# kmaninis/OSVOS-PyTorch

Measured on AMD Instinct MI355X. Metric: frames/sec (fwd+bwd) OSVOS-VGG16 854x480 per GPU; mask IoU vs ref, higher is better.
Workload: dtype f32 (3x bf16-split operands on MFMA, f32 accumulate); 1 GPU; 854x480 batch=1 online fine-tune loop (train_online.py), fused-head loss, nAveGrad=5, SGD 8-group, fp32x3, frame resident in HBM; global_batch=1, parallelism=dp1, grad_allreduce=none, rccl_ranks_seen=1

## Files before the change

### osvos-pytorch_amd/csrc/conv3x3_f32x3.hip

```cpp
#include "common.h"
#include "kernels.h"
#include "epi.h"
#include "maskbits.h"
#include "h2split.h"

namespace {

typedef __bf16 bf16x8_t __attribute__((ext_vector_type(8)));
typedef __bf16 bf16x2_t __attribute__((ext_vector_type(2)));
typedef unsigned int u32x4 __attribute__((ext_vector_type(4)));

struct ConvArgsX {
  const float* x;
  const float* wpk;
  const uint4* wpk3;
  const float* bias;
  const float* mask;
  float* y;
  int N, H, W, Cin, Cout, CoutP, y_cs;
  int tiles_x, tiles_y, nct;
  int relu, map, nsp;
  int ksplit;
  float* part;
  ConvEpi epi;
  int sk_order;
  unsigned* sk_tickets;
  float* sk_part;
};

constexpr int cdivx(int a, int b) { return (a + b - 1) / b; }
constexpr int pitch_x(int rbw, int hw) {
  return rbw == 32 ? hw : (rbw == 16 ? cdivx(hw, 16) * 16 : cdivx(hw - 8, 16) * 16 + 8);
}

template <int RBW_, int TBX_, int TBY_, int NB_, int WGM_, int WGN_, int OCC_, int ILV_ = 0>
struct CfgX {
  static constexpr int RBW = RBW_, TBX = TBX_, TBY = TBY_, NB = NB_, WGM = WGM_, WGN = WGN_, OCC = OCC_;
  static constexpr int ILV = ILV_;
  static constexpr int RBH = 32 / RBW;
  static constexpr int TW = TBX * RBW, TH = TBY * RBH;
  static constexpr int HWD = TW + 2, HHT = TH + 2;
  static constexpr int PITCH = pitch_x(RBW, HWD);
  static constexpr int PLANE = HHT * PITCH;
  static constexpr int BN = NB * 32;
  static constexpr int A_U4 = 6 * PLANE;
  static constexpr int B_ITEMS = 18 * BN;
  static constexpr int B_U4 = 3 * B_ITEMS;
  static constexpr int BUF_U4 = A_U4 + B_U4;
  static constexpr int A_ITEMS = HHT * HWD * 2;
  static constexpr int NT = 64 * WGM * WGN;
  static constexpr int NA = cdivx(A_ITEMS, NT);
  static constexpr int NBL = cdivx(B_ITEMS, NT);
  static constexpr int MB = TBX * TBY;
  static constexpr int WM = MB / WGM, WN = NB / WGN;
  static constexpr size_t LDS_BYTES = (size_t)(BUF_U4 + 2) * 16;
  static constexpr int A_U4_2 = 4 * PLANE, B_U4_2 = 2 * B_ITEMS;
  static constexpr size_t LDS_BYTES_2 = (size_t)(A_U4_2 + B_U4_2 + 2 + 4) * 16;
  static constexpr int SK_SLOT_F4 = NT * WM * WN * 4;
  static constexpr int ROW_U4 = 18 * BN;
  static constexpr size_t LDS_BYTES_PIPE = (size_t)(2 * A_U4 + 2 * ROW_U4 + 2) * 16;
  static_assert(WGM * WGN == 4 || WGM * WGN == 8, "4 or 8 waves per workgroup");
  static_assert(MB % WGM == 0 && NB % WGN == 0, "wave grid must divide the tile");
  static_assert(LDS_BYTES <= 160 * 1024, "tile does not fit the 160 KB LDS of a gfx950 CU");
};

__device__ inline unsigned cvt2(float a, float b) {
  bf16x2_t h;
  h[0] = (__bf16)a;
  h[1] = (__bf16)b;
  return __builtin_bit_cast(unsigned, h);
}
__device__ inline void split2(float a, float b, unsigned& p0, unsigned& p1, unsigned& p2) {
  p0 = cvt2(a, b);
  float ra = a - __uint_as_float(p0 << 16), rb = b - __uint_as_float(p0 & 0xffff0000u);
  p1 = cvt2(ra, rb);
  ra -= __uint_as_float(p1 << 16);
  rb -= __uint_as_float(p1 & 0xffff0000u);
  p2 = cvt2(ra, rb);
}
__device__ inline void split8(const u32x4& lo, const u32x4& hi, uint4& p0, uint4& p1, uint4& p2) {
  const f32x4 a = __builtin_bit_cast(f32x4, lo), b = __builtin_bit_cast(f32x4, hi);
  split2(a[0], a[1], p0.x, p1.x, p2.x);
  split2(a[2], a[3], p0.y, p1.y, p2.y);
  split2(b[0], b[1], p0.z, p1.z, p2.z);
  split2(b[2], b[3], p0.w, p1.w, p2.w);
}

__device__ inline void split8_hm(const u32x4& lo, const u32x4& hi, uint4& p0, uint4& p1) {
  const f32x4 a = __builtin_bit_cast(f32x4, lo), b = __builtin_bit_cast(f32x4, hi);
  auto two = [](float x, float y, unsigned& q0, unsigned& q1) {
    q0 = cvt2(x, y);
    q1 = cvt2(x - __uint_as_float(q0 << 16), y - __uint_as_float(q0 & 0xffff0000u));
  };
  two(a[0], a[1], p0.x, p1.x);
  two(a[2], a[3], p0.y, p1.y);
  two(b[0], b[1], p0.z, p1.z);
  two(b[2], b[3], p0.w, p1.w);
}

template <class C, int PS, int SK, int NP = 3, int HP = 0, int PIPE = 0>
__global__ __launch_bounds__(C::NT, C::OCC) void conv3x3_f32x3_kernel(ConvArgsX a) {
  static_assert(NP == 2 || NP == 3, "two or three bf16 pieces per operand");
  static_assert(HP == 0 || (NP == 2 && PS == 1 && SK == 0), "h2: two pieces, pre-split pack, plain grid");
  static_assert(PIPE == 0 || (PS == 1 && NP == 3 && HP == 0 && C::ILV != 0 && C::NT == 512), "pipelined loop: pre-split three-piece eight-wave tiles");
  extern __shared__ __attribute__((aligned(16))) char smem[];
  uint4* As = reinterpret_cast<uint4*>(smem);
  uint4* Bs = As + (NP == 3 ? C::A_U4 : C::A_U4_2);
  const int tid = threadIdx.x, lane = tid & 63, wave = tid >> 6;
  const int li = lane & 31, lh = lane >> 5;
  const int wm = wave / C::WGN, wn = wave % C::WGN;
  const int nch_all = a.Cin >> 4;

  unsigned u = 0, u_end = 0, vme = 0, sk_U = 0, my_first_tile = 0;
  if constexpr (SK != 0) {
    const unsigned G = gridDim.x;
    vme = (G & 7u) == 0 ? (blockIdx.x & 7u) * (G >> 3) + (blockIdx.x >> 3) : blockIdx.x;
    sk_U = (unsigned)(a.nct * a.nsp) * (unsigned)nch_all;
    u = (unsigned)(((unsigned long long)vme * sk_U) / G);
    u_end = (unsigned)(((unsigned long long)(vme + 1) * sk_U) / G);
    my_first_tile = u / (unsigned)nch_all;
  }
 for (;;) {
  int sp, ct;
  int kc_begin, kc_end;
  unsigned tile_id = 0;
  if constexpr (SK != 0) {
    if (u >= u_end) break;
    tile_id = u / (unsigned)nch_all;
    kc_begin = (int)(u - tile_id * (unsigned)nch_all);
    kc_end = min(nch_all, kc_begin + (int)(u_end - u));
    if (a.sk_order == 0) { sp = (int)(tile_id / (unsigned)a.nct); ct = (int)(tile_id % (unsigned)a.nct); }
    else { ct = (int)(tile_id / (unsigned)a.nsp); sp = (int)(tile_id % (unsigned)a.nsp); }
  } else {
    if (a.map == 0) {
      sp = blockIdx.x / a.nct;
      ct = blockIdx.x % a.nct;
    } else {
      const int j = blockIdx.x >> 3;
      ct = j % a.nct;
      sp = (j / a.nct) * 8 + (blockIdx.x & 7);
      if (sp >= a.nsp) return;
    }
    kc_begin = (int)((long)nch_all * blockIdx.y / a.ksplit);
    kc_end = (int)((long)nch_all * (blockIdx.y + 1) / a.ksplit);
  }
  const int tx = sp % a.tiles_x;
  sp /= a.tiles_x;
  const int ty = sp % a.tiles_y;
  const int n = sp / a.tiles_y;
  const int x0 = tx * C::TW, y0 = ty * C::TH, co0 = ct * C::BN;
  const int CQ = a.Cin >> 2;
  const float* ximg = a.x + (size_t)n * a.H * a.W * a.Cin;

  constexpr unsigned OOB = 0x80000000u;
  const __amdgpu_buffer_rsrc_t xrs = __builtin_amdgcn_make_buffer_rsrc(const_cast<float*>(ximg), 0, (int)((size_t)a.H * a.W * a.Cin * 4), 0x00020000);
  const __amdgpu_buffer_rsrc_t wrs = __builtin_amdgcn_make_buffer_rsrc(const_cast<float*>(a.wpk), 0, (int)((size_t)9 * CQ * a.CoutP * 16), 0x00020000);
  unsigned a_off[C::NA];
  int a_dst[C::NA];
#pragma unroll
  for (int i = 0; i < C::NA; ++i) {
    const int e = tid + i * C::NT;
    const int g = e & 1, pix = e >> 1;
    const int hy = pix / C::HWD, hx = pix % C::HWD;
    const int gy = y0 + hy - 1, gx = x0 + hx - 1;
    const bool slot = e < C::A_ITEMS;
    a_dst[i] = slot ? g * C::PLANE + hy * C::PITCH + hx : -1;
    a_off[i] = (slot && gy >= 0 && gy < a.H && gx >= 0 && gx < a.W) ? (unsigned)(((gy * a.W + gx) * a.Cin + 8 * g) * 4) : OOB;
  }
  constexpr int NBI = PS ? cdivx(NP * C::B_ITEMS, C::NT) : C::NBL;
  constexpr int TPI = C::NT / (2 * C::BN);
  static_assert(!PS || C::NT % (2 * C::BN) == 0, "pre-split staging: the thread block must cover whole (piece, tap) rows");
  unsigned b_off[PS ? 1 : C::NBL];
  unsigned b_step = 0;
  int b_row0 = 0;
  if (PS) {
    const int CG = a.Cin >> 3;
    b_row0 = tid / (2 * C::BN);
    const int rem = tid % (2 * C::BN), g = rem / C::BN, nn = rem % C::BN;
    b_off[0] = (co0 + nn < a.CoutP) ? (unsigned)(((b_row0 * CG + g) * a.CoutP + co0 + nn) * 16) : OOB;
    b_step = (unsigned)(TPI * CG * a.CoutP * 16);
  } else {
#pragma unroll
    for (int i = 0; i < C::NBL; ++i) {
      const int e = tid + i * C::NT;
      const int tap = e / (2 * C::BN), rem = e % (2 * C::BN);
      const int g = rem / C::BN, nn = rem % C::BN;
      b_off[i] = (e < C::B_ITEMS && co0 + nn < a.CoutP) ? (unsigned)(((tap * CQ + 2 * g) * a.CoutP + co0 + nn) * 16) : OOB;
    }
  }
  const unsigned b_q1 = (unsigned)a.CoutP * 16u;
  const __amdgpu_buffer_rsrc_t w3rs = __builtin_amdgcn_make_buffer_rsrc(const_cast<uint4*>(PS ? a.wpk3 : reinterpret_cast<const uint4*>(a.wpk)), 0,
                                                                        PS ? (int)((size_t)27 * (a.Cin >> 3) * a.CoutP * 16) : 0, 0x00020000);

  u32x4 ra[C::NA][2], rb[NBI][PS ? 1 : 2];
  auto load_item = [&](int it, int kc) {
    if (it < C::NA) {
      ra[it][0] = __builtin_amdgcn_raw_buffer_load_b128(xrs, a_off[it], kc * 64, 0);
      ra[it][1] = __builtin_amdgcn_raw_buffer_load_b128(xrs, a_off[it] + 16u, kc * 64, 0);
    } else if (it < C::NA + NBI) {
      const int i = it - C::NA;
      if constexpr (PS != 0) {
        const unsigned off = (b_row0 + i * TPI < 9 * NP) ? b_off[0] : OOB;
        rb[i][0] = __builtin_amdgcn_raw_buffer_load_b128(w3rs, off, kc * 2 * a.CoutP * 16 + i * b_step, 0);
      } else {
        rb[i][0] = __builtin_amdgcn_raw_buffer_load_b128(wrs, b_off[i], kc * 4 * a.CoutP * 16, 0);
        rb[i][1] = __builtin_amdgcn_raw_buffer_load_b128(wrs, b_off[i] + b_q1, kc * 4 * a.CoutP * 16, 0);
      }
    }
  };
  auto load_chunk = [&](int kc) {
#pragma unroll
    for (int it = 0; it < C::NA + NBI; ++it) load_item(it, kc);
  };
  static_assert(!C::ILV || C::NA + NBI <= 9 * C::WM, "interleaved staging: one item per step must cover the chunk");
  int h2_ea = kH2NoScale;
  float h2_sc = 1.f;
  unsigned* const h2_mx = reinterpret_cast<unsigned*>(As + C::A_U4_2 + C::B_U4_2 + 2);
  static_assert(HP == 0 || C::NT <= 512, "h2: exchange slots");
  auto store_chunk = [&]() {
#pragma unroll
    for (int i = 0; i < C::NA; ++i) {
      uint4 p0, p1, p2;
      if constexpr (HP != 0) h2_split8(ra[i][0], ra[i][1], h2_sc, p0, p1);
      else if constexpr (NP == 3) split8(ra[i][0], ra[i][1], p0, p1, p2);
      else split8_hm(ra[i][0], ra[i][1], p0, p1);
      if (C::A_ITEMS % C::NT == 0 || a_dst[i] >= 0) {
        As[a_dst[i]] = p0;
        As[a_dst[i] + 2 * C::PLANE] = p1;
        if constexpr (NP == 3) As[a_dst[i] + 4 * C::PLANE] = p2;
      }
    }
    if constexpr (PS != 0) {
#pragma unroll
      for (int i = 0; i < NBI; ++i) {
        const int e3 = tid + i * C::NT;
        if ((NP * C::B_ITEMS) % C::NT == 0 || e3 < NP * C::B_ITEMS) Bs[e3] = __builtin_bit_cast(uint4, rb[i][0]);
      }
    } else {
#pragma unroll
      for (int i = 0; i < NBI; ++i) {
        uint4 p0, p1, p2;
        if constexpr (NP == 3) split8(rb[i][0], rb[i][1], p0, p1, p2);
        else split8_hm(rb[i][0], rb[i][1], p0, p1);
        const int e = tid + i * C::NT;
        if (C::B_ITEMS % C::NT == 0 || e < C::B_ITEMS) {
          Bs[e] = p0;
          Bs[e + C::B_ITEMS] = p1;
          if constexpr (NP == 3) Bs[e + 2 * C::B_ITEMS] = p2;
        }
      }
    }
  };

  int a_idx[C::WM];
#pragma unroll
  for (int mi = 0; mi < C::WM; ++mi) {
    const int mb = wm * C::WM + mi;
// ... 45 lines not shown
    }
#if defined(OSVOS_X3_ABL) && OSVOS_X3_ABL == 4
    if (kc == kc_begin)
#endif
    store_chunk();
#if !(defined(OSVOS_X3_ABL) && OSVOS_X3_ABL == 5)
    __syncthreads();
#endif
    const bool more = kc + 1 < kc_end;
    if (!C::ILV && more) load_chunk(kc + 1);
    uint4 fb[2][3][C::WN], fa[2][3];
    auto ldB = [&](int tap, int set) {
#if defined(OSVOS_X3_ABL) && OSVOS_X3_ABL == 2
      if (tap > 0) return;
#endif
#pragma unroll
      for (int p = 0; p < NP; ++p)
#pragma unroll
        for (int ni = 0; ni < C::WN; ++ni) fb[set][p][ni] = Bs[b_idx + (p * 9 + tap) * 2 * C::BN + ni * 32];
    };
    auto ldA = [&](int tap, int mi, int set) {
#if defined(OSVOS_X3_ABL) && OSVOS_X3_ABL == 2
      if (tap > 0 || mi > 1) return;
#endif
      const int r = tap / 3, s = tap % 3;
#pragma unroll
      for (int p = 0; p < NP; ++p) fa[set][p] = As[a_idx[mi] + p * 2 * C::PLANE + r * C::PITCH + s];
    };
    ldB(0, 0);
    ldA(0, 0, 0);
#pragma unroll
    for (int tap = 0; tap < 9; ++tap) {
#pragma unroll
      for (int mi = 0; mi < C::WM; ++mi) {
        const int step = tap * C::WM + mi;
        if (mi + 1 < C::WM) ldA(tap, mi + 1, (step + 1) & 1);
        else if (tap + 1 < 9) ldA(tap + 1, 0, (step + 1) & 1);
        if (mi == 0 && tap + 1 < 9) ldB(tap + 1, (tap + 1) & 1);
#if !(defined(OSVOS_X3_ABL) && OSVOS_X3_ABL == 3)
        if (C::ILV && more) load_item(step, kc + 1);
#endif
        __builtin_amdgcn_sched_barrier(0);
        const int sa = step & 1, sb = tap & 1;
        constexpr int NPROD = NP == 3 ? 6 : 3;
        constexpr int PB[6] = {NP == 3 ? 2 : 1, NP == 3 ? 0 : 0, NP == 3 ? 1 : 0, 1, 0, 0};
        constexpr int PA[6] = {NP == 3 ? 0 : 0, NP == 3 ? 2 : 1, NP == 3 ? 1 : 0, 0, 1, 0};
#pragma unroll
        for (int t = 0; t < NPROD; ++t)
#pragma unroll
          for (int ni = 0; ni < C::WN; ++ni)
#if defined(OSVOS_X3_ABL) && OSVOS_X3_ABL == 1
            acc[mi][ni][t] += __uint_as_float(fb[sb][PB[t]][ni].x ^ fb[sb][PB[t]][ni].w ^ fa[sa][PA[t]].x ^ fa[sa][PA[t]].w);
#else
            if constexpr (HP != 0)
              acc[mi][ni] = __builtin_amdgcn_mfma_f32_32x32x16_f16(__builtin_bit_cast(f16x8_t, fb[sb][PB[t]][ni]),
                                                                   __builtin_bit_cast(f16x8_t, fa[sa][PA[t]]), acc[mi][ni], 0, 0, 0);
            else
              acc[mi][ni] = __builtin_amdgcn_mfma_f32_32x32x16_bf16(__builtin_bit_cast(bf16x8_t, fb[sb][PB[t]][ni]),
                                                                    __builtin_bit_cast(bf16x8_t, fa[sa][PA[t]]), acc[mi][ni], 0, 0, 0);
#endif
        __builtin_amdgcn_sched_barrier(0);
      }
    }
  }
  } else {
    static_assert(C::NA == 2 && 3 * C::WM >= 4, "pipelined loop: two activation items per thread, four staging steps in a tap row");
    constexpr int NW = C::NT / 64;
    constexpr int NRI = C::ROW_U4 / 64;
    constexpr int NRW = cdivx(NRI, NW);
    static_assert(C::BN % 64 == 0, "pipelined loop: whole 64-slot DMA runs");
    uint4* const Bring = As + 2 * C::A_U4;
    typedef int i32x4 __attribute__((ext_vector_type(4)));
    const int CG = a.Cin >> 3;
    const unsigned long long wp = reinterpret_cast<unsigned long long>(a.wpk3);
    const i32x4 w3dma = {(int)(unsigned)wp, (int)(unsigned)(wp >> 32), (int)((size_t)27 * CG * a.CoutP * 16), 0x00020000};
    const int wv = __builtin_amdgcn_readfirstlane(wave);
    const unsigned lds_ring = (unsigned)(unsigned long long)(__attribute__((address_space(3))) char*)Bring;
    unsigned w_off[NRW];
#pragma unroll
    for (int d = 0; d < NRW; ++d) {
      const int i = wv + NW * d, run = i / (C::BN / 64), nn = (i % (C::BN / 64)) * 64 + lane;
      const int p = run / 6, s = (run >> 1) % 3, g = run & 1;
      w_off[d] = (i < NRI && co0 + nn < a.CoutP) ? (unsigned)((((p * 9 + s) * CG + g) * a.CoutP + co0 + nn) * 16) : OOB;
    }
#pragma clang diagnostic push
#pragma clang diagnostic ignored "-Winline-asm"
    auto dma_row = [&](int j) {
      const int kc = kc_begin + j / 3, r = j % 3;
      const int soff = (3 * r * CG + 2 * kc) * a.CoutP * 16;
      const unsigned base = lds_ring + (unsigned)((j & 1) * C::ROW_U4 * 16);
#pragma unroll
      for (int d = 0; d < NRW; ++d)
        if (NRI % NW == 0 || d + 1 < NRW || wv + NW * d < NRI)
          asm volatile("s_mov_b32 m0, %0\n\ts_nop 0\n\tbuffer_load_dwordx4 %1, %2, %3 offen lds"
                       : : "s"(base + (unsigned)((wv + NW * d) * 1024)), "v"(w_off[d]), "s"(w3dma), "s"(soff) : "m0", "memory");
    };
#pragma clang diagnostic pop
#if defined(OSVOS_X3_ABL) && OSVOS_X3_ABL == 5
#define X3P_BARRIER(ra_behind) asm volatile("s_waitcnt vmcnt(0) lgkmcnt(0)" ::: "memory")
#else
#define X3P_BARRIER(ra_behind) do { if (ra_behind) asm volatile("s_waitcnt vmcnt(4) lgkmcnt(0)\n\ts_barrier" ::: "memory"); \
                                    else asm volatile("s_waitcnt vmcnt(0) lgkmcnt(0)\n\ts_barrier" ::: "memory"); } while (0)
#endif
    auto ld_a = [&](int kc) {
#pragma unroll
      for (int i = 0; i < C::NA; ++i) {
        ra[i][0] = __builtin_amdgcn_raw_buffer_load_b128(xrs, a_off[i], kc * 64, 0);
        ra[i][1] = __builtin_amdgcn_raw_buffer_load_b128(xrs, a_off[i] + 16u, kc * 64, 0);
      }
    };
    auto put_a = [&](int i, uint4* Ab) {
      uint4 p0, p1, p2;
      split8(ra[i][0], ra[i][1], p0, p1, p2);
      if (C::A_ITEMS % C::NT == 0 || a_dst[i] >= 0) {
        Ab[a_dst[i]] = p0;
        Ab[a_dst[i] + 2 * C::PLANE] = p1;
        Ab[a_dst[i] + 4 * C::PLANE] = p2;
      }
    };
    static_assert((3 * C::WM) % 2 == 0, "pipelined loop: a tap row's steps must leave the A fragment set parity where it started");
    uint4 fb[3][3][C::WN], fa[2][3];
    auto ldB = [&](const uint4* Bc, int rr, int s) {
#if defined(OSVOS_X3_ABL) && OSVOS_X3_ABL == 2
      if (rr + s > 0) return;
#endif
#pragma unroll
      for (int p = 0; p < 3; ++p)
#pragma unroll
        for (int ni = 0; ni < C::WN; ++ni) fb[s][p][ni] = Bc[b_idx + (p * 3 + s) * 2 * C::BN + ni * 32];
    };
    auto ldA = [&](const uint4* Ac, int rr, int s, int mi, int set) {
#if defined(OSVOS_X3_ABL) && OSVOS_X3_ABL == 2
      if (rr + s > 0 || mi > 1) return;
#endif
#pragma unroll
      for (int p = 0; p < 3; ++p) fa[set][p] = Ac[a_idx[mi] + p * 2 * C::PLANE + rr * C::PITCH + s];
    };
    asm volatile("s_waitcnt lgkmcnt(0)\n\ts_barrier" ::: "memory");
    dma_row(0);
    ld_a(kc_begin);
    put_a(0, As);
    put_a(1, As);
    bool ra_behind = kc_begin + 1 < kc_end;
    if (ra_behind) ld_a(kc_begin + 1);
    X3P_BARRIER(ra_behind);
    ra_behind = false;
    ldB(Bring, 0, 0);
    ldA(As, 0, 0, 0, 0);
    for (int kc = kc_begin; kc < kc_end; ++kc) {
      const int buf = (kc - kc_begin) & 1;
      const uint4* const Acur = As + buf * C::A_U4;
      uint4* const Anext = As + (buf ^ 1) * C::A_U4;
      const bool more = kc + 1 < kc_end, more2 = kc + 2 < kc_end;
#pragma unroll
      for (int r = 0; r < 3; ++r) {
        const int j = 3 * (kc - kc_begin) + r;
        const uint4* const Bcur = Bring + (j & 1) * C::ROW_U4;
        const uint4* const Bnxt = Bring + ((j + 1) & 1) * C::ROW_U4;
        const bool dma_next = r < 2 || more;
#pragma unroll
        for (int s = 0; s < 3; ++s) {
#pragma unroll
          for (int mi = 0; mi < C::WM; ++mi) {
            const int step = s * C::WM + mi;
            if (mi + 1 < C::WM) ldA(Acur, r, s, mi + 1, (step + 1) & 1);
            else if (s + 1 < 3) ldA(Acur, r, s + 1, 0, (step + 1) & 1);
            if (mi == 0 && s + 1 < 3) ldB(Bcur, r, s + 1);
            if (r == 0) {
#if !(defined(OSVOS_X3_ABL) && OSVOS_X3_ABL == 4)
              if (step < 2 && more) put_a(step, Anext);
#endif
#if !(defined(OSVOS_X3_ABL) && OSVOS_X3_ABL == 3)
              if (step == 2 && dma_next) dma_row(j + 1);
              if (step == 3 && more2) { ld_a(kc + 2); ra_behind = true; }
#endif
            } else {
#if !(defined(OSVOS_X3_ABL) && OSVOS_X3_ABL == 3)
              if (step == 0 && dma_next) dma_row(j + 1);
#endif
            }
            if (step == 3 * C::WM - 1 && dma_next) {
              X3P_BARRIER(ra_behind);
              ra_behind = false;
              ldB(Bnxt, (r + 1) % 3, 0);
              ldA(r == 2 ? Anext : Acur, (r + 1) % 3, 0, 0, 0);
            }
            __builtin_amdgcn_sched_barrier(0);
            const int sa = step & 1, sb = s;
            constexpr int PB[6] = {2, 0, 1, 1, 0, 0};
            constexpr int PA[6] = {0, 2, 1, 0, 1, 0};
#pragma unroll
            for (int t = 0; t < 6; ++t)
#pragma unroll
              for (int ni = 0; ni < C::WN; ++ni)
#if defined(OSVOS_X3_ABL) && OSVOS_X3_ABL == 1
                acc[mi][ni][t] += __uint_as_float(fb[sb][PB[t]][ni].x ^ fb[sb][PB[t]][ni].w ^ fa[sa][PA[t]].x ^ fa[sa][PA[t]].w);
#else
                acc[mi][ni] = __builtin_amdgcn_mfma_f32_32x32x16_bf16(__builtin_bit_cast(bf16x8_t, fb[sb][PB[t]][ni]),
                                                                      __builtin_bit_cast(bf16x8_t, fa[sa][PA[t]]), acc[mi][ni], 0, 0, 0);
#endif
            __builtin_amdgcn_sched_barrier(0);
          }
        }
      }
    }
#undef X3P_BARRIER
  }

  if constexpr (HP != 0) {
    const unsigned wbits = reinterpret_cast<const unsigned*>(a.wpk3 + (size_t)2 * 9 * (a.Cin >> 3) * a.CoutP)[0];
    const int dl = -(h2_ea + h2_exp(wbits));
#pragma unroll
    for (int mi = 0; mi < C::WM; ++mi)
#pragma unroll
      for (int ni = 0; ni < C::WN; ++ni)
#pragma unroll
        for (int r = 0; r < 16; ++r) acc[mi][ni][r] = __builtin_ldexpf(acc[mi][ni][r], dl);
  }
  if constexpr (SK != 0) {
    u += (unsigned)(kc_end - kc_begin);
    if (!(kc_begin == 0 && kc_end == nch_all)) {
      const unsigned G = gridDim.x, nch = (unsigned)nch_all;
      const unsigned vf = ((tile_id * nch + 1u) * G - 1u) / sk_U;
      const unsigned vl = ((tile_id + 1u) * nch * G - 1u) / sk_U;
      const unsigned nparts = vl - vf + 1u, cme = vme - vf;
      constexpr int SC1 = 16;
      const __amdgpu_buffer_rsrc_t prs = __builtin_amdgcn_make_buffer_rsrc(a.sk_part, 0, (int)((size_t)G * 2 * C::SK_SLOT_F4 * 16), 0x00020000);
      unsigned* const flag = reinterpret_cast<unsigned*>(As + (PIPE ? 2 * C::A_U4 + 2 * C::ROW_U4 : C::BUF_U4) + 1);
      if (tid == 0) *flag = __hip_atomic_load(a.sk_tickets + tile_id, __ATOMIC_RELAXED, __HIP_MEMORY_SCOPE_AGENT);
      __syncthreads();
      bool last = *flag == nparts - 1u;
      if (!last) {
        const unsigned mine = (2u * vme + (tile_id == my_first_tile ? 0u : 1u)) * (unsigned)(C::SK_SLOT_F4 * 16);
#pragma unroll
        for (int mi = 0; mi < C::WM; ++mi)
#pragma unroll
          for (int ni = 0; ni < C::WN; ++ni)
#pragma unroll
            for (int q = 0; q < 4; ++q) {
              const f32x4 v = {acc[mi][ni][4 * q], acc[mi][ni][4 * q + 1], acc[mi][ni][4 * q + 2], acc[mi][ni][4 * q + 3]};
              __builtin_amdgcn_raw_buffer_store_b128(__builtin_bit_cast(u32x4, v), prs, mine + (unsigned)((((mi * C::WN + ni) * 4 + q) * C::NT + tid) * 16), 0, SC1);
            }
        asm volatile("s_waitcnt vmcnt(0)" ::: "memory");
        __syncthreads();
        if (tid == 0) *flag = __hip_atomic_fetch_add(a.sk_tickets + tile_id, 1u, __ATOMIC_RELAXED, __HIP_MEMORY_SCOPE_AGENT);
        __syncthreads();
        last = *flag == nparts - 1u;
        if (!last) continue;
      }
      if (tid == 0) a.sk_tickets[tile_id] = 0u;
      f32x16 own[C::WM][C::WN];
#pragma unroll
      for (int mi = 0; mi < C::WM; ++mi)
#pragma unroll
        for (int ni = 0; ni < C::WN; ++ni) own[mi][ni] = acc[mi][ni];
      for (unsigned j = 0; j < nparts; ++j) {
        const bool is_me = j == cme;
        const unsigned vo = vf + j;
        const unsigned first_tile_o = (unsigned)(((unsigned long long)vo * sk_U) / G) / nch;
        const unsigned src = (2u * vo + (tile_id == first_tile_o ? 0u : 1u)) * (unsigned)(C::SK_SLOT_F4 * 16);
        f32x4 part[C::WM][C::WN][4];
#pragma unroll
        for (int mi = 0; mi < C::WM; ++mi)
#pragma unroll
          for (int ni = 0; ni < C::WN; ++ni)
#pragma unroll
            for (int q = 0; q < 4; ++q) {
              if (is_me) part[mi][ni][q] = f32x4{own[mi][ni][4 * q], own[mi][ni][4 * q + 1], own[mi][ni][4 * q + 2], own[mi][ni][4 * q + 3]};
              else part[mi][ni][q] = __builtin_bit_cast(f32x4, __builtin_amdgcn_raw_buffer_load_b128(prs, src + (unsigned)((((mi * C::WN + ni) * 4 + q) * C::NT + tid) * 16), 0, SC1));
            }
#pragma unroll
        for (int mi = 0; mi < C::WM; ++mi)
#pragma unroll
          for (int ni = 0; ni < C::WN; ++ni)
#pragma unroll
            for (int q = 0; q < 4; ++q)
#pragma unroll
              for (int e = 0; e < 4; ++e) acc[mi][ni][4 * q + e] = j == 0 ? part[mi][ni][q][e] : acc[mi][ni][4 * q + e] + part[mi][ni][q][e];
      }
    }
  }
  const size_t img_elems = (size_t)a.H * a.W * a.y_cs;
  const bool split = a.ksplit > 1;
  const int cs = split ? a.Cout : a.y_cs;
  const size_t out_elems = (size_t)a.H * a.W * cs;
  float* obase = split ? a.part + ((size_t)blockIdx.y * a.N + n) * out_elems : a.y + n * out_elems;
  const __amdgpu_buffer_rsrc_t yrs = __builtin_amdgcn_make_buffer_rsrc(obase, 0, (int)(out_elems * 4), 0x00020000);
  const bool use_mask = !split && a.mask != nullptr;
  const __amdgpu_buffer_rsrc_t mrs = __builtin_amdgcn_make_buffer_rsrc(const_cast<float*>(use_mask ? a.mask + n * img_elems : a.y), 0,
                                                                       use_mask ? (int)(img_elems * 4) : 0, 0x00020000);
  const bool use_mbits = !split && a.epi.mask_bits != nullptr, put_bits = !split && a.epi.y_bits != nullptr;
  const int bw = a.y_cs >> 5;
  const size_t img_words = (size_t)a.H * a.W * bw;
  const __amdgpu_buffer_rsrc_t mbrs = __builtin_amdgcn_make_buffer_rsrc(use_mbits ? (void*)const_cast<unsigned*>(a.epi.mask_bits + n * img_words) : (void*)a.y, 0,
                                                                        use_mbits ? (int)(img_words * 4) : 0, 0x00020000);
  const __amdgpu_buffer_rsrc_t ybrs = __builtin_amdgcn_make_buffer_rsrc(put_bits ? (void*)(a.epi.y_bits + n * img_words) : (void*)a.y, 0,
                                                                        put_bits ? (int)(img_words * 4) : 0, 0x00020000);
  const bool use_bias = !split && a.bias != nullptr;
  const __amdgpu_buffer_rsrc_t brs = __builtin_amdgcn_make_buffer_rsrc(const_cast<float*>(use_bias ? a.bias : a.y), 0, use_bias ? a.Cout * 4 : 0, 0x00020000);
  const bool relu = !split && a.relu;
  float* const anyf = const_cast<float*>(a.wpk != nullptr ? a.wpk : reinterpret_cast<const float*>(a.wpk3));
  const bool pool_fwd = !split && a.epi.pooled != nullptr;
  const int PHo = (a.H + 1) / 2, PWo = (a.W + 1) / 2;
  const size_t poimg = (size_t)PHo * PWo * a.y_cs;
  const __amdgpu_buffer_rsrc_t pors = __builtin_amdgcn_make_buffer_rsrc(pool_fwd ? a.epi.pooled + n * poimg : anyf, 0, pool_fwd ? (int)(poimg * 4) : 0, 0x00020000);
#pragma unroll
  for (int ni = 0; ni < C::WN; ++ni) {
    const int cb = co0 + (wn * C::WN + ni) * 32 + 4 * lh;
    f32x4 bv[4];
#pragma unroll
    for (int q = 0; q < 4; ++q) bv[q] = __builtin_bit_cast(f32x4, __builtin_amdgcn_raw_buffer_load_b128(brs, (cb + 8 * q) * 4, 0, 0));
    f32x4 keep[C::WM][4];
#pragma unroll
    for (int mi = 0; mi < C::WM; ++mi) {
      const int mb = wm * C::WM + mi;
      const int oy = y0 + (mb / C::TBX) * C::RBH + li / C::RBW;
      const int ox = x0 + (mb % C::TBX) * C::RBW + li % C::RBW;
      const bool inside = oy < a.H && ox < a.W;
      const unsigned pix = inside ? (unsigned)((oy * a.W + ox) * cs) * 4u : OOB;
      const unsigned bitoff = (inside && cb - 4 * lh < a.Cout) ? (unsigned)(oy * a.W + ox) * (unsigned)(bw * 4) + (unsigned)((cb - 4 * lh) >> 5) * 4u : OOB;
      const unsigned mword = mb_load(mbrs, bitoff);
      unsigned ybits = 0;
#pragma unroll
      for (int q = 0; q < 4; ++q) {
        const int co = cb + 8 * q;
        const unsigned off = co < a.Cout ? pix + (unsigned)co * 4u : OOB;
        f32x4 v;
#pragma unroll
        for (int e = 0; e < 4; ++e) {
          v[e] = acc[mi][ni][4 * q + e] + bv[q][e];
          if (relu) v[e] = v[e] > 0.f ? v[e] : 0.f;
        }
        if (use_mbits) {
#pragma unroll
          for (int e = 0; e < 4; ++e) v[e] = mb_test(mword, q, lh, e) ? v[e] : 0.f;
        } else if (use_mask) {
          const f32x4 m = __builtin_bit_cast(f32x4, __builtin_amdgcn_raw_buffer_load_b128(mrs, off, 0, 0));
#pragma unroll
          for (int e = 0; e < 4; ++e) v[e] = m[e] > 0.f ? v[e] : 0.f;
        }
        ybits |= mb_bits_f32(v, q);
        __builtin_amdgcn_raw_buffer_store_b128(__builtin_bit_cast(u32x4, v), yrs, off, 0, 0);
        if (pool_fwd) {
#pragma unroll
          for (int e = 0; e < 4; ++e) keep[mi][q][e] = inside ? v[e] : 0.f;
        }
      }
      if (put_bits) mb_store(ybrs, bitoff, ybits, lh);
    }
    if (pool_fwd) {
      constexpr int NPW = C::RBW == 32 ? C::WM / 2 : C::WM;
#pragma unroll
      for (int j = 0; j < NPW; ++j) {
        const int mb = wm * C::WM + (C::RBW == 32 ? 2 * j : j);
        const int oy = y0 + (mb / C::TBX) * C::RBH, ox = x0 + (mb % C::TBX) * C::RBW + li % C::RBW;
        const bool writer = (li & 1) == 0 && (C::RBW == 32 || li < 16) && oy < a.H && ox < a.W;
        const unsigned ppix = writer ? (unsigned)(((oy >> 1) * PWo + (ox >> 1)) * a.y_cs) * 4u : OOB;
#pragma unroll
        for (int q = 0; q < 4; ++q) {
          const int co = cb + 8 * q;
          f32x4 m;
#pragma unroll
          for (int e = 0; e < 4; ++e) {
            float t;
            if constexpr (C::RBW == 32) {
              t = fmaxf(keep[2 * j][q][e], keep[2 * j + 1][q][e]);
            } else {
              t = keep[j][q][e];
              t = fmaxf(t, __shfl_xor(t, 16, 64));
            }
            m[e] = fmaxf(t, __shfl_xor(t, 1, 64));
          }
          __builtin_amdgcn_raw_buffer_store_b128(__builtin_bit_cast(u32x4, m), pors, (co < a.Cout && ppix != OOB) ? ppix + (unsigned)co * 4u : OOB, 0, 0);
        }
      }
    }
  }
  if constexpr (SK == 0) break;
 }
}

constexpr int kSkMaxGrid = 256, kSkMaxTiles = 8192;
constexpr size_t kSkSlotBytes = 128 * 1024;
constexpr size_t kSkTicketBytes = (size_t)kSkMaxTiles * 4;

template <class C, int PS, int SK, int NP = 3, int HP = 0, int PIPE = 0>
int launch_x2(const ConvArgsX& a0, int sk_grid, hipStream_t stream) {
  constexpr size_t lds_bytes = PIPE ? C::LDS_BYTES_PIPE : (NP == 3 ? C::LDS_BYTES : C::LDS_BYTES_2);
  static_assert(lds_bytes <= 160 * 1024, "tile does not fit the 160 KB LDS of a gfx950 CU");
  if (int rc = osvos_set_dyn_lds_once<&conv3x3_f32x3_kernel<C, PS, SK, NP, HP, PIPE>>(lds_bytes)) return rc;
  ConvArgsX a = a0;
  a.tiles_x = ceil_div(a.W, C::TW);
  a.tiles_y = ceil_div(a.H, C::TH);
  a.nct = ceil_div(a.CoutP, C::BN);
  a.nsp = a.tiles_x * a.tiles_y * a.N;
  if constexpr (SK != 0) {
    static_assert((size_t)C::SK_SLOT_F4 * 16 <= kSkSlotBytes, "stream-K partial slot larger than the workspace's");
    const long ntiles = (long)a.nct * a.nsp, units = ntiles * (a.Cin >> 4);
    OSVOS_ARG_CHECK(sk_grid > 0 && sk_grid <= kSkMaxGrid && ntiles <= kSkMaxTiles && units >= sk_grid && a.sk_tickets && a.sk_part && a.ksplit == 1,
                    "conv3x3 f32x3 stream-K: %ld tiles, %ld units on %d workgroups", ntiles, units, sk_grid);
    hipLaunchKernelGGL((conv3x3_f32x3_kernel<C, PS, SK, NP, HP, PIPE>), dim3((unsigned)sk_grid), dim3(C::NT), lds_bytes, stream, a);
  } else {
    const long blocks = a.map == 0 ? (long)a.nct * a.nsp : (long)a.nct * ((a.nsp + 7) / 8) * 8;
    OSVOS_ARG_CHECK(blocks > 0 && blocks < (1L << 31), "conv3x3 f32x3: grid of %ld blocks", blocks);
    hipLaunchKernelGGL((conv3x3_f32x3_kernel<C, PS, SK, NP, HP, PIPE>), dim3((unsigned)blocks, (unsigned)a.ksplit), dim3(C::NT), lds_bytes, stream, a);
  }
  OSVOS_LAUNCH_CHECK();
  return 0;
}
template <class C>
constexpr bool kPs2 = C::ILV != 0 && (C::NT == 512 || C::NT == 256);
template <class C>
constexpr bool kPs3 = C::ILV != 0 && C::NT == 512;
template <class C, bool SKT = false, bool PIPE = false>
int launch_x(const ConvArgsX& a, const ConvPlan& p, int pieces, hipStream_t stream) {
  if constexpr (kPs2<C>) {
    if (p.presplit && pieces == 22) return launch_x2<C, 1, 0, 2, 1>(a, 0, stream);
    if (p.presplit && pieces == 2) return launch_x2<C, 1, 0, 2>(a, 0, stream);
  }
  if (pieces == 2) return launch_x2<C, 0, 0, 2>(a, 0, stream);
  if constexpr (kPs3<C>) {
    if (p.presplit) {
      if constexpr (PIPE) {
        if (p.pipe) {
          if constexpr (SKT) {
            if (p.sk_grid > 0) return launch_x2<C, 1, 1, 3, 0, 1>(a, p.sk_grid, stream);
          }
          return launch_x2<C, 1, 0, 3, 0, 1>(a, 0, stream);
        }
      }
      if constexpr (SKT) {
        if (p.sk_grid > 0) return launch_x2<C, 1, 1>(a, p.sk_grid, stream);
      }
      return launch_x2<C, 1, 0>(a, 0, stream);
    }
  }
  return launch_x2<C, 0, 0>(a, 0, stream);
}

struct TileInfoX {
  int tw, th, bn, nt;
  size_t lds;
  bool ps2, ps3, skt, pipe;
  int (*launch)(const ConvArgsX&, const ConvPlan&, int, hipStream_t);
};

using X0 = CfgX<32, 1, 8, 4, 2, 2, 1>;
using X1 = CfgX<32, 1, 8, 4, 4, 2, 1>;
using X2 = CfgX<32, 1, 4, 4, 2, 2, 1>;
using X3 = CfgX<32, 1, 8, 2, 2, 2, 1>;
using X4 = CfgX<32, 1, 8, 2, 4, 2, 1>;
using X5 = CfgX<32, 1, 4, 2, 2, 2, 2>;
using X6 = CfgX<16, 1, 4, 2, 2, 2, 1>;
using X7 = CfgX<16, 1, 8, 2, 2, 2, 1>;
using X8 = CfgX<16, 1, 8, 2, 4, 2, 1>;
using X9 = CfgX<16, 1, 4, 4, 2, 2, 1>;
using X10 = CfgX<32, 1, 8, 4, 4, 2, 1, 1>;
using X11 = CfgX<32, 1, 8, 4, 2, 2, 1, 1>;
using X12 = CfgX<32, 1, 8, 2, 4, 2, 1, 1>;
using X13 = CfgX<32, 1, 4, 2, 2, 2, 2, 1>;
using X14 = CfgX<16, 1, 8, 2, 4, 2, 1, 1>;
using X15 = CfgX<32, 1, 8, 1, 8, 1, 1, 1>;
using X16 = CfgX<32, 1, 16, 2, 8, 1, 1, 1>;
using X17 = CfgX<16, 1, 16, 2, 8, 1, 1, 1>;
template <class C, bool SKT = false, bool PIPE = false>
constexpr TileInfoX infoX() { return TileInfoX{C::TW, C::TH, C::BN, C::NT, C::LDS_BYTES, kPs2<C>, kPs3<C>, SKT, PIPE, &launch_x<C, SKT, PIPE>}; }
constexpr TileInfoX kTilesX[] = {infoX<X0>(), infoX<X1>(), infoX<X2>(), infoX<X3>(), infoX<X4>(),
                                 infoX<X5>(), infoX<X6>(), infoX<X7>(), infoX<X8>(), infoX<X9>(),
                                 infoX<X10, true, true>(), infoX<X11>(), infoX<X12, true, true>(), infoX<X13>(), infoX<X14, true, true>(),
                                 infoX<X15>(), infoX<X16>(), infoX<X17>()};
constexpr int kNumTilesX = sizeof(kTilesX) / sizeof(kTilesX[0]);

long tiles_of(const TileInfoX& t, int N, int H, int W, int CoutP) {
  return (long)N * ceil_div(H, t.th) * ceil_div(W, t.tw) * ceil_div(CoutP, t.bn);
}

int pick_tile_x(int N, int H, int W, int CoutP) {
  const bool narrow = (long)ceil_div(W, 32) * 32 * 100 > (long)ceil_div(W, 16) * 16 * 110;
  if (CoutP <= 32) return 15;
  if (CoutP >= 128 && !narrow && tiles_of(kTilesX[10], N, H, W, CoutP) >= 200) return 10;
  return narrow ? 14 : 12;
}

int pick_ksplit_x(const TileInfoX& t, int N, int H, int W, int Cin, int Cout, int CoutP) {
  if (Cin < 256) return 1;
  const long blocks = tiles_of(t, N, H, W, CoutP);
  int ks = 1;
  while (ks < 8 && blocks * ks < 200 && (Cin / 16) / (ks * 2) >= 4) ks *= 2;
  return ks;
}

int choose(const ConvCall& c, ConvPlan* p) {
  const int N = c.N, H = c.H, W = c.W, Cin = c.Cin, Cout = c.Cout, y_cs = c.y_cs, CoutP = osvos_cout_pad(Cout);
  int tile = c.tile;
  const bool pool_fwd = c.pooled != nullptr;
  OSVOS_ARG_CHECK(c.x && (c.wpk || c.wpk3) && c.y, "conv3x3 f32x3: null pointer");
  OSVOS_ARG_CHECK(!pool_fwd || (c.relu && Cout % 4 == 0 && y_cs == Cout), "conv3x3 f32x3: fused pool forward needs ReLU and a dense Cout %% 4 == 0 result");
  OSVOS_ARG_CHECK(N > 0 && H > 0 && W > 0 && Cin > 0 && Cout > 0, "conv3x3 f32x3: bad shape");
  OSVOS_ARG_CHECK(osvos_conv3x3_f32x3_applicable(Cin, Cout, y_cs), "conv3x3 f32x3: needs Cin %% 16 == 0 (%d), y_cs %% 4 == 0 and >= Cout rounded up to 4 (%d, %d)",
                  Cin, Cout, y_cs);
  OSVOS_ARG_CHECK(Cout % 4 == 0 || (c.bias == nullptr && c.mask == nullptr), "conv3x3 f32x3: ragged Cout (%d) takes no bias / mask", Cout);
  OSVOS_ARG_CHECK(y_cs >= Cout, "conv3x3 f32x3: y channel stride %d < Cout %d", y_cs, Cout);
  OSVOS_ARG_CHECK((long)H * W * Cin < (1L << 29) && (long)H * W * y_cs < (1L << 29), "conv3x3 f32x3: image too large for 31-bit byte offsets");
  if (tile < 0) {
    OSVOS_ENV_INT(env_tile, "OSVOS_X3_TILE", -1);
    tile = env_tile >= 0 ? env_tile : pick_tile_x(N, H, W, CoutP);
    OSVOS_ENV_INT(wide2, "OSVOS_X2_TILE_FOR_10", 10);
    OSVOS_ENV_INT(mid2, "OSVOS_X2_TILE_FOR_12", 12);
    if (env_tile < 0 && c.pieces != 3 && !pool_fwd) tile = tile == 10 ? wide2 : (tile == 12 ? mid2 : tile);
    if (env_tile < 0 && (double)H * W * Cin > 27.0 * Cin * CoutP) tile += 100;
  }
  *p = ConvPlan();
  p->family = CONV_F32X3;
  p->map = tile >= 100 ? 1 : 0;
  tile %= 100;
  p->tile = tile;
  OSVOS_ARG_CHECK(tile >= 0 && tile < kNumTilesX, "conv3x3 f32x3: unknown tile config %d", tile);
  const TileInfoX& t = kTilesX[tile];
  if (c.part_ws != nullptr) {
    OSVOS_ENV_INT(env_ks, "OSVOS_X3_KSPLIT", 0);
    p->ksplit = c.ksplit > 0 ? c.ksplit : (env_ks > 0 && Cin >= 256 ? env_ks : pick_ksplit_x(t, N, H, W, Cin, Cout, CoutP));
    if (p->ksplit < 1 || p->ksplit > 8 || p->ksplit > (Cin >> 4) || Cout % 4 != 0) p->ksplit = 1;
  }
  if (c.mask_bits != nullptr || c.y_bits != nullptr)
    OSVOS_ARG_CHECK(Cout % 32 == 0 && y_cs == Cout, "conv3x3 f32x3: one-bit masks need a dense result with Cout %% 32 == 0 (Cout %d, stride %d)", Cout, y_cs);
  if (c.y_bits != nullptr) p->ksplit = 1;
  if (pool_fwd) {
    p->ksplit = 1;
    OSVOS_ARG_CHECK(tile == 10 || tile == 12 || tile == 14, "conv3x3 f32x3: fused pool forward is built for tiles 10, 12 and 14 (got %d)", tile);
  }
  if (c.sk_ws != nullptr && c.wpk3 != nullptr && t.skt && Cout % 4 == 0) {
    const long ntiles = tiles_of(t, N, H, W, CoutP), units = ntiles * (Cin >> 4);
    OSVOS_ENV_INT(env_grid, "OSVOS_X3_STREAMK_GRID", 0);
    OSVOS_ENV_INT(env_loss, "OSVOS_X3_STREAMK_MIN_LOSS", 6);
    int g = c.sk_grid > 0 ? c.sk_grid : (env_grid > 0 ? env_grid : osvos_cu_count());
    if (g > kSkMaxGrid) g = kSkMaxGrid;
    const long rounds = (ntiles * p->ksplit + g - 1) / g;
    const bool lossy = (tile == 12 || tile == 14) && (p->ksplit > 1 || (rounds * g - ntiles) * 100 >= (long)env_loss * rounds * g);
    if (ntiles <= kSkMaxTiles && units >= g && (c.sk_grid > 0 || lossy)) {
      p->sk_grid = g;
      p->ksplit = 1;
      p->sk_order = p->map ? 0 : 1;
      OSVOS_ENV_INT(env_order, "OSVOS_X3_STREAMK_ORDER", -1);
      if (env_order == 0 || env_order == 1) p->sk_order = env_order;
    }
  }
  if (c.pieces == 22) {
    OSVOS_ARG_CHECK(t.ps2 && c.wpk3 != nullptr,
                    "conv3x3 f32x3: the fp16-pair form is built for the pre-split eight-wave tiles (10, 12, 14, 15, 16, 17) with a pre-split pack");
    p->presplit = 1;
  } else {
    p->presplit = (c.pieces == 2 ? t.ps2 : t.ps3) && c.wpk3 != nullptr;
    OSVOS_ARG_CHECK(p->presplit || c.wpk != nullptr, "conv3x3 f32x3: this tile config has no pre-split form and no fp32 pack was given");
  }
  const bool three = c.pieces != 2 && c.pieces != 22;
  if (three && p->presplit && t.pipe) {
    OSVOS_ENV_INT(env_pipe, "OSVOS_X3_PIPE", 1);
    p->pipe = env_pipe != 0;
  }
  if (!three) p->sk_grid = p->sk_order = 0;
  return 0;
}

struct PackX3Table {
  const float* w[OSVOS_PACK_MAX];
  unsigned short* dst[OSVOS_PACK_MAX];
  int Cout[OSVOS_PACK_MAX], Cin[OSVOS_PACK_MAX], dgrad[OSVOS_PACK_MAX];
  unsigned char half[OSVOS_PACK_MAX];
  long start[OSVOS_PACK_MAX + 1];
  int n;
};

__device__ inline long pack_plane_elems(const PackX3Table& t, int k) {
  const int K = t.dgrad[k] ? t.Cout[k] : t.Cin[k], M = t.dgrad[k] ? t.Cin[k] : t.Cout[k];
  return 9L * (K / 8) * ((M + 31) / 32 * 32) * 8;
}
__global__ void wamax_zero_kernel(PackX3Table t) {
  const int k = (int)threadIdx.x;
  if (k < t.n && t.half[k]) *reinterpret_cast<unsigned*>(t.dst[k] + 2 * pack_plane_elems(t, k)) = 0u;
}
__global__ __launch_bounds__(256) void wamax_kernel(PackX3Table t) {
  const int k = (int)blockIdx.y;
  if (!t.half[k]) return;
  const long len = 9L * t.Cout[k] * t.Cin[k];
  const float* __restrict__ w = t.w[k];
  unsigned m = 0;
  for (long i = (long)blockIdx.x * 256 + threadIdx.x; i < len; i += (long)gridDim.x * 256) {
    const unsigned b = __float_as_uint(w[i]) & 0x7fffffffu;
    m = m > b ? m : b;
  }
  m = h2_wave_max(m);
  if ((threadIdx.x & 63) == 0 && m != 0u) atomicMax(reinterpret_cast<unsigned*>(t.dst[k] + 2 * pack_plane_elems(t, k)), m);
}

__global__ __launch_bounds__(256) void pack_x3_multi_kernel(PackX3Table t) {
  constexpr int ROW = 8 * 9 + 1;
  __shared__ float tile[32 * ROW];
  for (long blk = blockIdx.x; blk < t.start[t.n]; blk += gridDim.x) {
    int k = 0;
    while (blk >= t.start[k + 1]) ++k;
    const int dgrad = t.dgrad[k], Cout = t.Cout[k], Cin = t.Cin[k];
    const int K = dgrad ? Cout : Cin, M = dgrad ? Cin : Cout, MP = (M + 31) / 32 * 32, CG = K / 8;
    const long plane = 9L * CG * MP * 8;
    const int u = (int)(blk - t.start[k]);
    const int cg = u % CG, m0 = (u / CG) * 32;
    const float* __restrict__ w = t.w[k];
    const bool half = t.half[k] != 0;
    const float hsc = half ? h2_pow2(h2_exp(*reinterpret_cast<const unsigned*>(t.dst[k] + 2 * plane))) : 1.f;
    __syncthreads();
#pragma unroll
    for (int it = 0; it < 9; ++it) {
      const int L = it * 256 + (int)threadIdx.x;
      int ml, e, tap;
      float v = 0.f;
      if (dgrad) {
        e = L / 288;
        const int j = L % 288;
        ml = j / 9;
        tap = 8 - j % 9;
        if (m0 + ml < M) v = w[((long)(cg * 8 + e) * Cin + m0) * 9 + j];
      } else {
        ml = L / 72;
// ... 95 lines not shown
```

Before: 236.7 frames/s.

## Carry A-operand fragments across filter rows in pipelined conv3x3 loop

```diff
diff --git a/osvos-pytorch_amd/csrc/conv3x3_f32x3.hip b/osvos-pytorch_amd/csrc/conv3x3_f32x3.hip
--- a/osvos-pytorch_amd/csrc/conv3x3_f32x3.hip
+++ b/osvos-pytorch_amd/csrc/conv3x3_f32x3.hip
@@ -98,11 +98,13 @@
   two(b[2], b[3], p0.w, p1.w);
 }
 
-template <class C, int PS, int SK, int NP = 3, int HP = 0, int PIPE = 0>
+template <class C, int PS, int SK, int NP = 3, int HP = 0, int PIPE = 0, int CARRY = 0>
 __global__ __launch_bounds__(C::NT, C::OCC) void conv3x3_f32x3_kernel(ConvArgsX a) {
   static_assert(NP == 2 || NP == 3, "two or three bf16 pieces per operand");
   static_assert(HP == 0 || (NP == 2 && PS == 1 && SK == 0), "h2: two pieces, pre-split pack, plain grid");
   static_assert(PIPE == 0 || (PS == 1 && NP == 3 && HP == 0 && C::ILV != 0 && C::NT == 512), "pipelined loop: pre-split three-piece eight-wave tiles");
+  static_assert(CARRY == 0 || (PIPE == 1 && C::TBX == 1 && C::WM >= 2 && (C::RBW == 32 || C::RBW == 16)),
+                "row carry: pipelined loop, a wave's M blocks stacked vertically, RBH rows apart");
   extern __shared__ __attribute__((aligned(16))) char smem[];
   uint4* As = reinterpret_cast<uint4*>(smem);
   uint4* Bs = As + (NP == 3 ? C::A_U4 : C::A_U4_2);
@@ -454,6 +456,29 @@
       const uint4* const Acur = As + buf * C::A_U4;
       uint4* const Anext = As + (buf ^ 1) * C::A_U4;
       const bool more = kc + 1 < kc_end, more2 = kc + 2 < kc_end;
+      uint4 fc[CARRY ? C::RBH * (C::WM - 1) + 3 : 1][3][3];
+      auto carried = [](int rr, int mi) {
+        for (int m2 = mi + 1; m2 < C::WM; ++m2)
+          if (rr - C::RBH * (m2 - mi) >= 0) return true;
+        return false;
+      };
+      auto ldAc = [&](int rr, int s, int mi) {
+        if (carried(rr, mi)) return;
+        const int key = C::RBH * mi + rr;
+#if defined(OSVOS_X3_ABL) && OSVOS_X3_ABL == 2
+        if (rr + s > 0 || mi > 1) {
+#pragma unroll
+          for (int p = 0; p < 3; ++p) fc[key][s][p] = fc[mi == 0 ? 0 : C::RBH][0][p];
+          return;
+        }
+#endif
+#pragma unroll
+        for (int p = 0; p < 3; ++p) fc[key][s][p] = Acur[a_idx[mi] + p * 2 * C::PLANE + rr * C::PITCH + s];
+      };
+      if constexpr (CARRY != 0) {
+#pragma unroll
+        for (int p = 0; p < 3; ++p) fc[0][0][p] = fa[0][p];
+      }
 #pragma unroll
       for (int r = 0; r < 3; ++r) {
         const int j = 3 * (kc - kc_begin) + r;
@@ -465,8 +490,13 @@
 #pragma unroll
           for (int mi = 0; mi < C::WM; ++mi) {
             const int step = s * C::WM + mi;
-            if (mi + 1 < C::WM) ldA(Acur, r, s, mi + 1, (step + 1) & 1);
-            else if (s + 1 < 3) ldA(Acur, r, s + 1, 0, (step + 1) & 1);
+            if constexpr (CARRY != 0) {
+              if (mi + 1 < C::WM) ldAc(r, s, mi + 1);
+              else if (s + 1 < 3) ldAc(r, s + 1, 0);
+            } else {
+              if (mi + 1 < C::WM) ldA(Acur, r, s, mi + 1, (step + 1) & 1);
+              else if (s + 1 < 3) ldA(Acur, r, s + 1, 0, (step + 1) & 1);
+            }
             if (mi == 0 && s + 1 < 3) ldB(Bcur, r, s + 1);
             if (r == 0) {
 #if !(defined(OSVOS_X3_ABL) && OSVOS_X3_ABL == 4)
@@ -485,10 +515,19 @@
               X3P_BARRIER(ra_behind);
               ra_behind = false;
               ldB(Bnxt, (r + 1) % 3, 0);
-              ldA(r == 2 ? Anext : Acur, (r + 1) % 3, 0, 0, 0);
+              if constexpr (CARRY != 0) {
+                if (r == 2) ldA(Anext, 0, 0, 0, 0);
+                else ldAc(r + 1, 0, 0);
+              } else {
+                ldA(r == 2 ? Anext : Acur, (r + 1) % 3, 0, 0, 0);
+              }
             }
             __builtin_amdgcn_sched_barrier(0);
             const int sa = step & 1, sb = s;
+            auto af = [&](int p) -> const uint4& {
+              if constexpr (CARRY != 0) return fc[C::RBH * mi + r][s][p];
+              else return fa[sa][p];
+            };
             constexpr int PB[6] = {2, 0, 1, 1, 0, 0};
             constexpr int PA[6] = {0, 2, 1, 0, 1, 0};
 #pragma unroll
@@ -496,10 +535,10 @@
 #pragma unroll
               for (int ni = 0; ni < C::WN; ++ni)
 #if defined(OSVOS_X3_ABL) && OSVOS_X3_ABL == 1
-                acc[mi][ni][t] += __uint_as_float(fb[sb][PB[t]][ni].x ^ fb[sb][PB[t]][ni].w ^ fa[sa][PA[t]].x ^ fa[sa][PA[t]].w);
+                acc[mi][ni][t] += __uint_as_float(fb[sb][PB[t]][ni].x ^ fb[sb][PB[t]][ni].w ^ af(PA[t]).x ^ af(PA[t]).w);
 #else
                 acc[mi][ni] = __builtin_amdgcn_mfma_f32_32x32x16_bf16(__builtin_bit_cast(bf16x8_t, fb[sb][PB[t]][ni]),
-                                                                      __builtin_bit_cast(bf16x8_t, fa[sa][PA[t]]), acc[mi][ni], 0, 0, 0);
+                                                                      __builtin_bit_cast(bf16x8_t, af(PA[t])), acc[mi][ni], 0, 0, 0);
 #endif
             __builtin_amdgcn_sched_barrier(0);
           }
@@ -686,11 +725,11 @@
 constexpr size_t kSkSlotBytes = 128 * 1024;
 constexpr size_t kSkTicketBytes = (size_t)kSkMaxTiles * 4;
 
-template <class C, int PS, int SK, int NP = 3, int HP = 0, int PIPE = 0>
+template <class C, int PS, int SK, int NP = 3, int HP = 0, int PIPE = 0, int CARRY = 0>
 int launch_x2(const ConvArgsX& a0, int sk_grid, hipStream_t stream) {
   constexpr size_t lds_bytes = PIPE ? C::LDS_BYTES_PIPE : (NP == 3 ? C::LDS_BYTES : C::LDS_BYTES_2);
   static_assert(lds_bytes <= 160 * 1024, "tile does not fit the 160 KB LDS of a gfx950 CU");
-  if (int rc = osvos_set_dyn_lds_once<&conv3x3_f32x3_kernel<C, PS, SK, NP, HP, PIPE>>(lds_bytes)) return rc;
+  if (int rc = osvos_set_dyn_lds_once<&conv3x3_f32x3_kernel<C, PS, SK, NP, HP, PIPE, CARRY>>(lds_bytes)) return rc;
   ConvArgsX a = a0;
   a.tiles_x = ceil_div(a.W, C::TW);
   a.tiles_y = ceil_div(a.H, C::TH);
@@ -701,11 +740,11 @@
     const long ntiles = (long)a.nct * a.nsp, units = ntiles * (a.Cin >> 4);
     OSVOS_ARG_CHECK(sk_grid > 0 && sk_grid <= kSkMaxGrid && ntiles <= kSkMaxTiles && units >= sk_grid && a.sk_tickets && a.sk_part && a.ksplit == 1,
                     "conv3x3 f32x3 stream-K: %ld tiles, %ld units on %d workgroups", ntiles, units, sk_grid);
-    hipLaunchKernelGGL((conv3x3_f32x3_kernel<C, PS, SK, NP, HP, PIPE>), dim3((unsigned)sk_grid), dim3(C::NT), lds_bytes, stream, a);
+    hipLaunchKernelGGL((conv3x3_f32x3_kernel<C, PS, SK, NP, HP, PIPE, CARRY>), dim3((unsigned)sk_grid), dim3(C::NT), lds_bytes, stream, a);
   } else {
     const long blocks = a.map == 0 ? (long)a.nct * a.nsp : (long)a.nct * ((a.nsp + 7) / 8) * 8;
     OSVOS_ARG_CHECK(blocks > 0 && blocks < (1L << 31), "conv3x3 f32x3: grid of %ld blocks", blocks);
-    hipLaunchKernelGGL((conv3x3_f32x3_kernel<C, PS, SK, NP, HP, PIPE>), dim3((unsigned)blocks, (unsigned)a.ksplit), dim3(C::NT), lds_bytes, stream, a);
+    hipLaunchKernelGGL((conv3x3_f32x3_kernel<C, PS, SK, NP, HP, PIPE, CARRY>), dim3((unsigned)blocks, (unsigned)a.ksplit), dim3(C::NT), lds_bytes, stream, a);
   }
   OSVOS_LAUNCH_CHECK();
   return 0;
@@ -714,7 +753,7 @@
 constexpr bool kPs2 = C::ILV != 0 && (C::NT == 512 || C::NT == 256);
 template <class C>
 constexpr bool kPs3 = C::ILV != 0 && C::NT == 512;
-template <class C, bool SKT = false, bool PIPE = false>
+template <class C, bool SKT = false, bool PIPE = false, int CARRY0 = 0, int CARRY1 = 0>
 int launch_x(const ConvArgsX& a, const ConvPlan& p, int pieces, hipStream_t stream) {
   if constexpr (kPs2<C>) {
     if (p.presplit && pieces == 22) return launch_x2<C, 1, 0, 2, 1>(a, 0, stream);
@@ -726,9 +765,9 @@
       if constexpr (PIPE) {
         if (p.pipe) {
           if constexpr (SKT) {
-            if (p.sk_grid > 0) return launch_x2<C, 1, 1, 3, 0, 1>(a, p.sk_grid, stream);
+            if (p.sk_grid > 0) return launch_x2<C, 1, 1, 3, 0, 1, CARRY1>(a, p.sk_grid, stream);
           }
-          return launch_x2<C, 1, 0, 3, 0, 1>(a, 0, stream);
+          return launch_x2<C, 1, 0, 3, 0, 1, CARRY0>(a, 0, stream);
         }
       }
       if constexpr (SKT) {
@@ -765,11 +804,11 @@
 using X15 = CfgX<32, 1, 8, 1, 8, 1, 1, 1>;
 using X16 = CfgX<32, 1, 16, 2, 8, 1, 1, 1>;
 using X17 = CfgX<16, 1, 16, 2, 8, 1, 1, 1>;
-template <class C, bool SKT = false, bool PIPE = false>
-constexpr TileInfoX infoX() { return TileInfoX{C::TW, C::TH, C::BN, C::NT, C::LDS_BYTES, kPs2<C>, kPs3<C>, SKT, PIPE, &launch_x<C, SKT, PIPE>}; }
+template <class C, bool SKT = false, bool PIPE = false, int CARRY0 = 0, int CARRY1 = 0>
+constexpr TileInfoX infoX() { return TileInfoX{C::TW, C::TH, C::BN, C::NT, C::LDS_BYTES, kPs2<C>, kPs3<C>, SKT, PIPE, &launch_x<C, SKT, PIPE, CARRY0, CARRY1>}; }
 constexpr TileInfoX kTilesX[] = {infoX<X0>(), infoX<X1>(), infoX<X2>(), infoX<X3>(), infoX<X4>(),
                                  infoX<X5>(), infoX<X6>(), infoX<X7>(), infoX<X8>(), infoX<X9>(),
-                                 infoX<X10, true, true>(), infoX<X11>(), infoX<X12, true, true>(), infoX<X13>(), infoX<X14, true, true>(),
+                                 infoX<X10, true, true, 1, 0>(), infoX<X11>(), infoX<X12, true, true, 1, 1>(), infoX<X13>(), infoX<X14, true, true, 0, 0>(),
                                  infoX<X15>(), infoX<X16>(), infoX<X17>()};
 constexpr int kNumTilesX = sizeof(kTilesX) / sizeof(kTilesX[0]);
 
```

After: 238.1 frames/s (median of 6 runs). No clear change (+0.6%).
